# barry-mir/mixing-style-transfer

Hardware: AMD Instinct MI355X
Metric: triplets/sec (10 s @ 44.1 kHz, 4-stem, bs=24) (higher is better)
Workload: dtype f32

## Files before the change

include/mst.h:

```cpp
#ifndef MST_H_
#define MST_H_

#include <stddef.h>
#include <stdint.h>

#ifdef __cplusplus
extern "C" {
#endif

#define MST_ABI_VERSION 1

#define MST_OK 0
#define MST_EINVAL (-1)
#define MST_ENOMEM (-2)
#define MST_EHIP (-3)

int mst_version(void);
const char* mst_last_error(void);

typedef struct mst_plan mst_plan;

int mst_plan_create(mst_plan** out, int sample_rate, int n_fft, int hop, int n_mels,
                    const float* window, const float* fb, int detailed_bins);
void mst_plan_destroy(mst_plan* plan);
int mst_plan_frames(const mst_plan* plan, int T);
int mst_plan_feature_dim(const mst_plan* plan);
size_t mst_melfeat_workspace_bytes(const mst_plan* plan, int B, int T);

int mst_melfeat_forward(const mst_plan* plan, const float* stems, int B, int T, float* logmel,
                        float* feats, void* workspace, size_t workspace_bytes, void* stream);
int mst_melfeat_forward_stems(const mst_plan* plan, const float* const stems4[4], long long clip_stride,
                              int B, int T, float* logmel, float* feats, void* workspace,
                              size_t workspace_bytes, void* stream);
int mst_melfeat_forward_pcm16(const mst_plan* plan, const int16_t* stems, int B, int T, float* logmel,
                              float* feats, void* workspace, size_t workspace_bytes, void* stream);
int mst_melfeat_forward_stems_pcm16(const mst_plan* plan, const int16_t* const stems4[4], long long clip_stride,
                                    int B, int T, float* logmel, float* feats, void* workspace,
                                    size_t workspace_bytes, void* stream);

#define MST_LOGMEL_REF 0
#define MST_LOGMEL_CM32 1
#define MST_LOGMEL_CM16 2
int mst_plan_layout_supported(const mst_plan* plan, int layout);
typedef struct mst_melfeat_io {
  const void* stems4[4];
  long long clip_stride;
  int32_t pcm16;
  int32_t layout;
  void* logmel;
  void* logmel_lo;
  uint32_t* absmax;
  float* feats;
} mst_melfeat_io;
int mst_melfeat_forward_io(const mst_plan* plan, const mst_melfeat_io* io, int B, int T, void* workspace,
                           size_t workspace_bytes, void* stream);

typedef struct mst_encoder mst_encoder;

typedef struct mst_encoder_config {
  int32_t n_mels, split_size, overlap, n_subbands;
  int32_t feature_dim, embed_dim;
  int32_t film_hidden;
  int32_t attn_hidden;
  float bn_eps;
} mst_encoder_config;

// ... 177 lines not shown
```

mixing-style-transfer_amd/_lib.py:

```python
import ctypes as C
import os
import subprocess
import threading

_HERE = os.path.dirname(os.path.abspath(__file__))
LIB_PATH = os.environ.get("MST_LIB", os.path.join(_HERE, "libmst.so"))
CSRC = os.path.join(_HERE, "csrc")

MST_OK = 0


class MstError(RuntimeError):
    pass


class EncoderConfig(C.Structure):
    _fields_ = [("n_mels", C.c_int32), ("split_size", C.c_int32), ("overlap", C.c_int32),
                ("n_subbands", C.c_int32), ("feature_dim", C.c_int32), ("embed_dim", C.c_int32),
                ("film_hidden", C.c_int32), ("attn_hidden", C.c_int32), ("bn_eps", C.c_float)]


_W_FIELDS = ["conv1_w", "conv1_b", "bn1_w", "bn1_b", "bn1_mean", "bn1_var",
             "conv2_w", "conv2_b", "bn2_w", "bn2_b", "bn2_mean", "bn2_var",
             "mlp0_w", "mlp0_b", "mlp3_w", "mlp3_b", "head_w", "head_b",
# ... 51 lines not shown

class FilmPtrs(C.Structure):
    _fields_ = [(k, C.c_void_p) for k in ("mlp0_w", "mlp0_b", "mlp3_w", "mlp3_b", "head_w", "head_b")]


SYMBOLS = {
    "mst_version": (C.c_int, []),
    "mst_last_error": (C.c_char_p, []),
    "mst_plan_create": (C.c_int, [C.POINTER(C.c_void_p), C.c_int, C.c_int, C.c_int, C.c_int, C.c_void_p, C.c_void_p,
                                  C.c_int]),
    "mst_plan_destroy": (None, [C.c_void_p]),
    "mst_plan_frames": (C.c_int, [C.c_void_p, C.c_int]),
    "mst_plan_feature_dim": (C.c_int, [C.c_void_p]),
    "mst_melfeat_workspace_bytes": (C.c_size_t, [C.c_void_p, C.c_int, C.c_int]),
    "mst_melfeat_forward": (C.c_int, [C.c_void_p, C.c_void_p, C.c_int, C.c_int, C.c_void_p, C.c_void_p, C.c_void_p,
                                      C.c_size_t, C.c_void_p]),
    "mst_melfeat_forward_stems": (C.c_int, [C.c_void_p, C.POINTER(C.c_void_p), C.c_longlong, C.c_int, C.c_int,
                                            C.c_void_p, C.c_void_p, C.c_void_p, C.c_size_t, C.c_void_p]),
    "mst_melfeat_forward_pcm16": (C.c_int, [C.c_void_p, C.c_void_p, C.c_int, C.c_int, C.c_void_p, C.c_void_p,
                                            C.c_void_p, C.c_size_t, C.c_void_p]),
    "mst_melfeat_forward_stems_pcm16": (C.c_int, [C.c_void_p, C.POINTER(C.c_void_p), C.c_longlong, C.c_int, C.c_int,
                                                  C.c_void_p, C.c_void_p, C.c_void_p, C.c_size_t, C.c_void_p]),
    "mst_plan_layout_supported": (C.c_int, [C.c_void_p, C.c_int]),
    "mst_melfeat_forward_io": (C.c_int, [C.c_void_p, C.POINTER(MelfeatIO), C.c_int, C.c_int, C.c_void_p, C.c_size_t,
                                         C.c_void_p]),
    "mst_encoder_layout_supported": (C.c_int, [C.c_void_p, C.c_int]),
    "mst_encoder_forward_in": (C.c_int, [C.c_void_p, C.POINTER(LogmelIn), C.c_int, C.c_void_p, C.c_int, C.c_void_p,
                                         C.POINTER(EncoderTaps), C.c_void_p, C.c_size_t, C.c_void_p]),
    "mst_encoder_create": (C.c_int, [C.POINTER(C.c_void_p), C.POINTER(EncoderConfig), C.POINTER(EncoderWeights)]),
    "mst_encoder_destroy": (None, [C.c_void_p]),
    "mst_encoder_set_precision": (C.c_int, [C.c_void_p, C.c_int]),
    "mst_encoder_set_train_precision": (C.c_int, [C.c_void_p, C.c_int]),
    "mst_encoder_workspace_bytes": (C.c_size_t, [C.c_void_p, C.c_int, C.c_int]),
    "mst_encoder_forward": (C.c_int, [C.c_void_p, C.c_void_p, C.c_int, C.c_void_p, C.c_int, C.c_void_p,
                                      C.POINTER(EncoderTaps), C.c_void_p, C.c_size_t, C.c_void_p]),
    "mst_encoder_train_workspace_bytes": (C.c_size_t, [C.c_void_p, C.c_int, C.c_int]),
    "mst_encoder_forward_train": (C.c_int, [C.c_void_p, C.c_void_p, C.c_int, C.c_void_p, C.c_int, C.c_void_p,
                                            C.POINTER(EncoderTrainTaps), C.c_void_p, C.c_size_t, C.c_void_p]),
    "mst_dropout_mask": (C.c_int, [C.c_float, C.c_uint64, C.c_longlong, C.c_void_p, C.c_void_p]),
    "mst_head_save_bytes": (C.c_size_t, [C.POINTER(HeadDims), C.c_int, C.c_float]),
    "mst_head_backward_workspace_bytes": (C.c_size_t, [C.POINTER(HeadDims), C.c_int]),
    "mst_head_forward_train": (C.c_int, [C.POINTER(HeadDims), C.POINTER(HeadPtrs), C.c_void_p, C.c_int, C.c_float, C.c_uint64, C.c_float,
                                         C.c_uint64, C.c_void_p, C.c_void_p, C.c_size_t, C.c_void_p]),
    "mst_head_backward": (C.c_int, [C.POINTER(HeadDims), C.POINTER(HeadPtrs), C.c_void_p, C.c_int, C.c_float, C.c_uint64, C.c_float,
                                    C.c_uint64, C.c_void_p, C.c_void_p, C.POINTER(HeadPtrs), C.c_void_p, C.c_void_p, C.c_size_t, C.c_void_p]),
    "mst_film_save_bytes": (C.c_size_t, [C.POINTER(FilmDims), C.c_int]),
# ... 88 lines not shown
```

mixing-style-transfer_amd/csrc/fft_pk.h:

```cpp
#pragma once
#include <hip/hip_runtime.h>

namespace mstpk {

typedef float v2f __attribute__((ext_vector_type(2)));
typedef float v4f __attribute__((ext_vector_type(4)));

__device__ __forceinline__ v2f mk(float x, float y) {
  v2f r;
  r.x = x, r.y = y;
  return r;
}
__device__ __forceinline__ v2f add_mi(v2f a, v2f b) {
  v2f d;
  asm("v_pk_add_f32 %0, %1, %2 op_sel:[0,1] op_sel_hi:[1,0] neg_hi:[0,1]" : "=v"(d) : "v"(a), "v"(b));
  return d;
}
__device__ __forceinline__ v2f sub_mi(v2f a, v2f b) {
  v2f d;
  asm("v_pk_add_f32 %0, %1, %2 op_sel:[0,1] op_sel_hi:[1,0] neg_lo:[0,1]" : "=v"(d) : "v"(a), "v"(b));
  return d;
}
__device__ __forceinline__ v2f cmul(v2f a, v2f w) {
  v2f t, d;
// ... 100 lines not shown
    v2f* dst = scr + 144 * (lane >> 4) + (lane & 15);
#pragma unroll
    for (int u = 0; u < 2; ++u)
#pragma unroll
      for (int t = 0; t < 8; ++t) dst[576 * u + 16 * t] = x[8 * u + t];
  }
  __builtin_amdgcn_wave_barrier();
  {
    const v2f* sa = scr + lane;
    const v2f* sb = scr + jb_of(lane);
#pragma unroll
    for (int t = 0; t < 8; ++t) x[t] = sa[144 * t], x[8 + t] = sb[144 * t];
    fill2();
#pragma unroll
    for (int t = 1; t < 8; ++t) {
      x[t] = cmul(x[t], tw3[(t - 1) * 64 + lane]);
      x[8 + t] = cmul(x[8 + t], tw3[(7 + t - 1) * 64 + lane]);
    }
    dft8(x);
    dft8(x + 8);
  }
}

inline void fill_twiddles_host(float2* tw2, float2* tw3) {
  const double pi = 3.14159265358979323846;
  for (int t = 1; t < 8; ++t)
    for (int lane = 0; lane < 64; ++lane) {
      const double a = -2.0 * pi * (double)((lane & 15) * t) / 128.0;
      tw2[(t - 1) * 64 + lane] = make_float2((float)cos(a), (float)sin(a));
      for (int u = 0; u < 2; ++u) {
        const int j = u ? (lane ? 128 - lane : 64) : lane;
        const double b = -2.0 * pi * (double)(j * t) / 1024.0;
        tw3[(u * 7 + t - 1) * 64 + lane] = make_float2((float)cos(b), (float)sin(b));
      }
    }
}

}
```

mixing-style-transfer_amd/csrc/melfeat.hip:

```cpp
#include "common.h"
#include "fft_wave.h"
#include "fft_pk.h"

#include <algorithm>
#include <cmath>
#include <vector>


namespace {

constexpr int kWaves = 8;
constexpr int kFPW = 2;
constexpr int kTF = kWaves * kFPW;
constexpr int kTileStride = kTF + 1;
constexpr int kThreads = kWaves * 64;
constexpr int nf_of(int n_fft) { return n_fft >= 2048 ? 1 : kFPW; }
constexpr int kNumScalars = 80;

enum : int {
  S_LOGSUM = 0,
  S_LINSUM = 4,
  S_MASK = 8,
  S_SQ = 12,
  S_PEAK = 20,
// ... 919 lines not shown
    hipError_t e = hipFuncSetAttribute(reinterpret_cast<const void*>(melfeat_kernel<NFFT, NB, ST>),
                                       hipFuncAttributeMaxDynamicSharedMemorySize, (int)lds);
    if (e != hipSuccess) return e;
  }
  hipLaunchKernelGGL((melfeat_kernel<NFFT, NB, ST>), dim3(grid), dim3(kThreads), lds, st, kp);
  return hipGetLastError();
}

template <int NFFT, typename ST, int WPS>
hipError_t launch_melfeat_spw(const KParams& kp, int grid, size_t lds, hipStream_t st) {
  {
    hipError_t e = hipFuncSetAttribute(reinterpret_cast<const void*>(melfeat_spw_kernel<NFFT, ST, WPS>),
                                       hipFuncAttributeMaxDynamicSharedMemorySize, (int)lds);
    if (e != hipSuccess) return e;
  }
  hipLaunchKernelGGL((melfeat_spw_kernel<NFFT, ST, WPS>), dim3(grid), dim3(SpwGeom<WPS>::THREADS), lds, st, kp);
  return hipGetLastError();
}

template <int NFFT>
constexpr int tw_count_of() { return FftPlan<NFFT / 2>::TW; }

#include "melfeat_v2.inc"
#include "melfeat_v2_2048.inc"

}

struct mst_plan {
  int sr, n_fft, hop, n_mels, detailed_bins, feat_dim;
  int nc, nb, nnz, tw_count;
  int glen[4], goff[4];
  int batches_per_run;
  float* d_window = nullptr;
  float2* d_tw = nullptr;
  float2* d_tw2 = nullptr;
  int tw2_count = 0;
  float2* d_post = nullptr;
  float* d_melw = nullptr;
  LaneBand* d_lanebands = nullptr;
  bool v2_ok = false;
  int v2_nslot = 0, v2_glen[kV2Slots] = {0}, v2_goff[kV2Slots] = {0}, v2_segw_count = 0, v2_wps = 3, v2_maxcnt = 1;
  int2* d_v2_bandtab = nullptr;
  bool v4_ok = false;
  int v4_nslot = 0, v4_glen[4] = {0, 0, 0, 0}, v4_goff[4] = {0, 0, 0, 0}, v4_segw_count = 0, v4_maxcnt = 0;
  float2* d_v4_tw4 = nullptr;
  float2* d_v4_segw = nullptr;
  int* d_v4_pstart = nullptr;
  int* d_v4_pid = nullptr;
  int* d_v4_bandtab = nullptr;
  float2* d_v2_tw2 = nullptr;
  float2* d_v2_tw3 = nullptr;
  float2* d_v2_segw = nullptr;
  int* d_v2_segstart = nullptr;
  int* d_v2_segid = nullptr;
};

namespace {

void add_pass_tw(std::vector<float2>& tw, int NC, int R, int NS) {
  if (NS == 1) return;
  const int nbf = NS <= 64 ? 1 : NC / R / 64;
  for (int u = 0; u < nbf; ++u)
    for (int t = 1; t < R; ++t)
      for (int lane = 0; lane < 64; ++lane) {
// ... 9 lines not shown
    case 512: return {{8, 1}, {8, 8}, {8, 64}};
    case 1024: return {{8, 1}, {8, 8}, {4, 64}, {4, 256}};
  }
  return {};
}

int frames_per_run_of(const mst_plan* p, int , int F) {
  if (p->batches_per_run > 0) return p->batches_per_run * kTF;
  int fpr = (F + 31) / 32;
  fpr += fpr & 1;
  return std::max(2 * kTF, fpr);
}
int runs_per_clip(const mst_plan* p, int B, int F) {
  const int fpr = frames_per_run_of(p, B, F);
  return (F + fpr - 1) / fpr;
}
int pstride_of(const mst_plan* p) { return 4 * p->n_mels + kNumScalars; }

int v2_fpw(const mst_plan* p, int F) { return std::max(1, ((F + 31) / 32 + p->v2_wps - 1) / p->v2_wps); }
int v2_runs(const mst_plan* p, int F) {
  const int fpr = p->v2_wps * v2_fpw(p, F);
  return (F + fpr - 1) / fpr;
}

bool segment_bins(const float* fb, int n_bins, int M, std::vector<int>& seg, std::vector<float>& wl, std::vector<float>& wh) {
  std::vector<int> peak(M, -1);
  for (int m = 0; m < M; ++m) {
    float best = 0.f;
    for (int k = 0; k < n_bins; ++k)
      if (fb[(size_t)k * M + m] > best) best = fb[(size_t)k * M + m], peak[m] = k;
  }
  seg.assign(n_bins, 0), wl.assign(n_bins, 0.f), wh.assign(n_bins, 0.f);
  int prev = 0;
  for (int k = 0; k < n_bins; ++k) {
    int b0 = -1, b1 = -1, cnt = 0;
    for (int m = 0; m < M; ++m)
      if (fb[(size_t)k * M + m] != 0.0f) {
        if (cnt == 0) b0 = m;
        b1 = m;
        ++cnt;
      }
    if (cnt > 2 || (cnt == 2 && b1 != b0 + 1)) return false;
    int s = prev;
    if (cnt == 2) {
      s = b1, wl[k] = fb[(size_t)k * M + b0], wh[k] = fb[(size_t)k * M + b1];
    } else if (cnt == 1) {
// ... 177 lines not shown
  if (melw.empty()) melw.push_back(0.f);
  std::vector<float2> tw;
  for (auto pr : passes_of(p->nc)) add_pass_tw(tw, p->nc, pr.first, pr.second);
  p->tw_count = (int)tw.size();
  std::vector<float2> tw2;
  if (n_fft <= 1024)
    for (auto pr : passes_of(n_fft)) add_pass_tw(tw2, n_fft, pr.first, pr.second);
  p->tw2_count = (int)tw2.size();
  if (tw2.empty()) tw2.push_back(make_float2(1.f, 0.f));
  std::vector<float2> post(p->nc);
  for (int q = 0; q < p->nc / 64; ++q)
    for (int lane = 0; lane < 64; ++lane) {
      const int k = lane + 64 * q;
      const double a = -2.0 * M_PI * (double)k / (double)n_fft;
      post[(size_t)q * 64 + lane] = make_float2((float)cos(a), (float)sin(a));
    }
  {
    std::vector<float2> segw, t2(mstpk::kTw2Rows * 64), t3(mstpk::kTw3Rows * 64);
    std::vector<int> segstart, segid;
    std::vector<int2> bandtab;
    const char* w = getenv("MST_V2_WPS");
    p->v2_wps = ((w && atoi(w) == 2) || n_mels > 128) ? 2 : 3;
    p->v2_ok = n_fft == 1024 && hop == 256 && v2_build_segments(p, fb, segw, segstart, segid, bandtab);
    if (p->v2_ok) {
      mstpk::fill_twiddles_host(t2.data(), t3.data());
      int rc2;
      if ((rc2 = mst::upload(&p->d_v2_tw2, t2.data(), t2.size())) || (rc2 = mst::upload(&p->d_v2_tw3, t3.data(), t3.size())) ||
          (rc2 = mst::upload(&p->d_v2_segw, segw.data(), segw.size())) ||
          (rc2 = mst::upload(&p->d_v2_segstart, segstart.data(), segstart.size())) ||
          (rc2 = mst::upload(&p->d_v2_segid, segid.data(), segid.size())) ||
          (rc2 = mst::upload(&p->d_v2_bandtab, bandtab.data(), bandtab.size()))) {
        mst_plan_destroy(p);
        return rc2;
      }
    }
  }
  {
    std::vector<float2> segw, t2(mstpk::kTw2Rows * 64), t3(mstpk::kTw3Rows * 64), t4(16 * 64);
    std::vector<int> pstart, pid, bandtab;
    p->v4_ok = n_fft == 2048 && hop == 512 && v4_build_pieces(p, fb, segw, pstart, pid, bandtab);
    if (p->v4_ok) {
      mstpk::fill_twiddles_host(t2.data(), t3.data());
      for (int t = 0; t < 8; ++t)
        for (int lane = 0; lane < 64; ++lane)
          for (int u = 0; u < 2; ++u) {
            const int k = (u ? (lane ? 128 - lane : 64) : lane) + 128 * t;
// ... 22 lines not shown
  }
  *out = p;
  return MST_OK;
}

void mst_plan_destroy(mst_plan* p) {
  if (!p) return;
  (void)hipFree(p->d_window), (void)hipFree(p->d_tw), (void)hipFree(p->d_tw2), (void)hipFree(p->d_post), (void)hipFree(p->d_melw),
      (void)hipFree(p->d_lanebands);
  (void)hipFree(p->d_v2_tw2), (void)hipFree(p->d_v2_tw3), (void)hipFree(p->d_v2_segw), (void)hipFree(p->d_v2_segstart),
      (void)hipFree(p->d_v2_segid), (void)hipFree(p->d_v2_bandtab);
  (void)hipFree(p->d_v4_tw4), (void)hipFree(p->d_v4_segw), (void)hipFree(p->d_v4_pstart), (void)hipFree(p->d_v4_pid),
      (void)hipFree(p->d_v4_bandtab);
  delete p;
}

int mst_plan_frames(const mst_plan* p, int T) { return p ? 1 + T / p->hop : MST_EINVAL; }
int mst_plan_feature_dim(const mst_plan* p) { return p ? p->feat_dim : MST_EINVAL; }

size_t mst_melfeat_workspace_bytes(const mst_plan* p, int B, int T) {
  if (!p || B <= 0 || T <= 0) return 0;
  const int F = 1 + T / p->hop;
  const int runs = std::max(runs_per_clip(p, B, F), p->v2_ok ? v2_runs(p, F) : (p->v4_ok ? v4_runs(F) : 0));
  return mst::align_up((size_t)B * runs * pstride_of(p) * sizeof(float), 256);
}

}

namespace {
struct LogmelOut {
  int layout = MST_LOGMEL_REF;
  void* lo = nullptr;
  unsigned* absmax = nullptr;
};
int melfeat_forward_impl(const mst_plan* p, const void* const stems4[4], bool pcm16, long long clip_stride, int B, int T,
                         float* logmel, float* feats, void* workspace, size_t workspace_bytes, void* stream,
                         const LogmelOut& lo = LogmelOut());
bool plan_uses_v2(const mst_plan* p);
}

extern "C" {

int mst_melfeat_forward(const mst_plan* p, const float* stems, int B, int T, float* logmel, float* feats,
                        void* workspace, size_t workspace_bytes, void* stream) {
  MST_REQUIRE(p && stems, "mst_melfeat_forward: NULL plan/stems");
  const void* four[4] = {stems, stems + 2 * (size_t)T, stems + 4 * (size_t)T, stems + 6 * (size_t)T};
  return melfeat_forward_impl(p, four, false, (long long)8 * T, B, T, logmel, feats, workspace, workspace_bytes, stream);
// ... 118 lines not shown
                        (size_t)v4::kWPS * v4::kBLK * 4 * 128 * sizeof(float) + 16;
    MST_REQUIRE(lds4 <= 160 * 1024, "mst_melfeat_forward: LDS %zu B exceeds 160 KiB", lds4);
    const int grid4 = B * k4.runs_per_clip;
    e = pcm16 ? launch_melfeat_v2_2048<short>(k4, grid4, lds4, st) : launch_melfeat_v2_2048<float>(k4, grid4, lds4, st);
  } else if (use_v2) {
    K2Params k2{};
    for (int i = 0; i < 4; ++i) k2.stem[i] = stems4[i];
    k2.clip_stride = clip_stride, k2.logmel = logmel, k2.partials = reinterpret_cast<float*>(workspace);
    k2.out_mode = lmo.layout, k2.logmel_lo = lmo.lo, k2.absmax = lmo.absmax;
    k2.window = p->d_window, k2.tw2 = p->d_v2_tw2, k2.tw3 = p->d_v2_tw3, k2.segw = p->d_v2_segw;
    k2.segstart = p->d_v2_segstart, k2.segid = p->d_v2_segid, k2.bandtab = p->d_v2_bandtab, k2.maxcnt = p->v2_maxcnt;
    k2.B = B, k2.T = T, k2.F = F, k2.M = p->n_mels;
    k2.nslot = p->v2_nslot, k2.segw_count = p->v2_segw_count;
    for (int r = 0; r < kV2Slots; ++r) k2.glen[r] = p->v2_glen[r], k2.goff[r] = p->v2_goff[r];
    k2.fpw = v2_fpw(p, F), k2.runs_per_clip = v2_runs(p, F), k2.pstride = pstride_of(p);
    kp.runs_per_clip = k2.runs_per_clip;
    const int wps = p->v2_wps;
    const bool wide = p->n_mels > 128;
    const size_t lds2 = (size_t)((mstpk::kTw2Rows + mstpk::kTw3Rows) * 64 + p->v2_segw_count + 4 * wps * mstpk::kScr) * sizeof(float2) +
                        (size_t)(wps * (wide ? 4 : (wps == 2 ? 8 : 4)) * 4 * (wide ? 256 : 128) + 1024) * sizeof(float) + 16;
    MST_REQUIRE(lds2 <= 160 * 1024, "mst_melfeat_forward: LDS %zu B exceeds 160 KiB", lds2);
    const int grid2 = B * k2.runs_per_clip;
    if (wide) e = pcm16 ? launch_melfeat_v2<short, 2, 4>(k2, grid2, lds2, st) : launch_melfeat_v2<float, 2, 4>(k2, grid2, lds2, st);
    else if (wps == 3) {
      const bool stdt = v2_table_is_standard(p) && !getenv("MST_V2_NOSTD");
      e = pcm16 ? launch_melfeat_v2<short, 3>(k2, grid2, lds2, st, stdt) : launch_melfeat_v2<float, 3>(k2, grid2, lds2, st, stdt);
    }
    else e = pcm16 ? launch_melfeat_v2<short, 2>(k2, grid2, lds2, st) : launch_melfeat_v2<float, 2>(k2, grid2, lds2, st);
  } else {
  const int grid = B * kp.runs_per_clip;
  const int wps = getenv("MST_SPW_WPS") ? atoi(getenv("MST_SPW_WPS")) : 3;
  auto spw_lds = [&](int w) {
    return (size_t)(nc + p->tw2_count + 4 * w * (p->n_fft + p->n_fft / 8)) * sizeof(float2) +
           (size_t)(((p->nnz + 3) & ~3) + (w == 2 ? 16 : 6) * (8 * p->n_mels + 1)) * sizeof(float);
  };
  const bool spw_ok = kp.vec_ok && kp.vec4_ok && p->hop * 4 == p->n_fft && p->n_mels <= 128 && p->nb == 2 &&
                      (p->n_fft == 512 || p->n_fft == 1024) && !getenv("MST_MELFEAT_GENERIC");
  const bool spw3 = spw_ok && wps == 3 && p->n_fft == 1024 && spw_lds(3) <= 160 * 1024;
  const bool spw = spw3 || (spw_ok && spw_lds(2) <= 160 * 1024);
  if (spw3) {
    e = pcm16 ? launch_melfeat_spw<1024, short, 3>(kp, grid, spw_lds(3), st) : launch_melfeat_spw<1024, float, 3>(kp, grid, spw_lds(3), st);
  } else if (spw) {
    const size_t lds_spw = spw_lds(2);
    if (p->n_fft == 1024)
      e = pcm16 ? launch_melfeat_spw<1024, short, 2>(kp, grid, lds_spw, st) : launch_melfeat_spw<1024, float, 2>(kp, grid, lds_spw, st);
    else
      e = pcm16 ? launch_melfeat_spw<512, short, 2>(kp, grid, lds_spw, st) : launch_melfeat_spw<512, float, 2>(kp, grid, lds_spw, st);
  } else {
#define MST_CASE(NF)                                                                                          \
// ... 26 lines not shown
```

mixing-style-transfer_amd/csrc/melfeat_v2.inc:

```

constexpr int kV2Slots = 6;

struct K2Params {
  const void* stem[4];
  long long clip_stride;
  float* logmel;
  void* logmel_lo;
  unsigned* absmax;
  int out_mode;
  float* partials;
  const float* window;
  const float2* tw2;
  const float2* tw3;
  const float2* segw;
  const int* segstart;
  const int* segid;
  const int2* bandtab;
  int B, T, F, M;
  int nslot, glen[kV2Slots], goff[kV2Slots], segw_count;
  int maxcnt;
  int fpw;
  int runs_per_clip, pstride;
};

namespace v2 {
using namespace mstpk;

constexpr int kP2 = 0;
constexpr int kExN = 288;
constexpr int kExDump = kExN - 1;
constexpr int kExHi = 544;
constexpr int kExLo = kExHi + kExN;
static_assert(kExLo + kExN <= kScr, "exchange areas must fit the FFT scratch");
// ... 401 lines not shown
```

mixing-style-transfer_amd/mixing_utils.py:

```python
import ctypes as C

import numpy as np
import torch

from . import _lib

STEMS = ("vocals", "bass", "drums", "other")

FEATURES_DEFERRED = -32768.0


def deferred_features(feature_dim: int) -> torch.Tensor:
    return torch.full((feature_dim,), FEATURES_DEFERRED, dtype=torch.float32)


def is_deferred(features: torch.Tensor) -> torch.Tensor:
    return features[..., :1] == FEATURES_DEFERRED


def detailed_bins_for_feature_dim(feature_dim: int):
    if feature_dim < 8 or (feature_dim - 8) % 4:
        return None
    sd = (feature_dim - 8) // 4 - 9
    if sd == 5:
# ... 15 lines not shown
    slope = hz.unsqueeze(0) - freqs.unsqueeze(1)
    lower = (-1.0 * slope[:, :-2]) / dhz[:-1]
    upper = slope[:, 2:] / dhz[1:]
    return torch.max(torch.zeros(1), torch.min(lower, upper))


class LogMel:

    def __init__(self, layout, data, lo=None, absmax=None):
        self.layout, self.data, self.lo, self.absmax = layout, data, lo, absmax
        self.B, self.frames, self.n_mels = data.shape[0], data.shape[1], data.shape[2]
        self.device = data.device

    def to_reference(self):
        if self.layout == _lib.LOGMEL_CM16 and self.lo is None:
            raise _lib.MstError("this LogMel holds the float16 HIGH parts only (what the plain-float16 kernels read): the fp32 "
                                "log-mel cannot be recovered from it -- ask stage A for the reference layout instead")
        x = self.data.float() if self.lo is None else self.data.float() + self.lo.float()
        return x.permute(0, 3, 2, 1).contiguous()


class MelFeatPlan:

    def __init__(self, sample_rate, n_fft, hop_length, n_mels, detailed_bins=0, window=None, fb=None):
        self.sample_rate, self.n_fft, self.hop_length, self.n_mels = sample_rate, n_fft, hop_length, n_mels
        self.window = (hann_window(n_fft) if window is None else window).detach().float().cpu().contiguous()
        self.fb = (melscale_fbanks_htk(n_fft // 2 + 1, n_mels, sample_rate) if fb is None else fb)
        self.fb = self.fb.detach().float().cpu().contiguous()
        h = C.c_void_p()
        L = _lib.lib()
        _lib.check(L.mst_plan_create(C.byref(h), sample_rate, n_fft, hop_length, n_mels,
                                     C.c_void_p(self.window.data_ptr()), C.c_void_p(self.fb.data_ptr()),
                                     int(detailed_bins)), "mst_plan_create")
        self._h = h
        self.feature_dim = L.mst_plan_feature_dim(h)
        self._ws = None

    def __del__(self):
        h, self._h = getattr(self, "_h", None), None
        if h:
            try:
                _lib.lib().mst_plan_destroy(h)
            except Exception:
                pass

    def frames(self, T: int) -> int:
        return 1 + T // self.hop_length

    def _workspace(self, B, T, device):
        need = _lib.lib().mst_melfeat_workspace_bytes(self._h, B, T)
        if self._ws is None or self._ws.numel() < need or self._ws.device != device:
            self._ws = torch.empty(need, dtype=torch.uint8, device=device)
        return self._ws, need

    def supports_layout(self, layout) -> bool:
        return bool(_lib.lib().mst_plan_layout_supported(self._h, int(layout)))

# ... 327 lines not shown
```

Before: 2772.

## Add paired-frame stage-A kernel splitting each run into sub-runs with a combine pass

```diff
diff --git a/include/mst.h b/include/mst.h
--- a/include/mst.h
+++ b/include/mst.h
@@ -42,6 +42,10 @@
 #define MST_LOGMEL_CM32 1
 #define MST_LOGMEL_CM16 2
 int mst_plan_layout_supported(const mst_plan* plan, int layout);
+
+#define MST_STAGE_A_PAIRS 0
+#define MST_STAGE_A_SINGLE 1
+int mst_plan_set_stage_a(mst_plan* plan, int kernel);
 typedef struct mst_melfeat_io {
   const void* stems4[4];
   long long clip_stride;
diff --git a/mixing-style-transfer_amd/_lib.py b/mixing-style-transfer_amd/_lib.py
--- a/mixing-style-transfer_amd/_lib.py
+++ b/mixing-style-transfer_amd/_lib.py
@@ -97,6 +97,7 @@
     "mst_melfeat_forward_stems_pcm16": (C.c_int, [C.c_void_p, C.POINTER(C.c_void_p), C.c_longlong, C.c_int, C.c_int,
                                                   C.c_void_p, C.c_void_p, C.c_void_p, C.c_size_t, C.c_void_p]),
     "mst_plan_layout_supported": (C.c_int, [C.c_void_p, C.c_int]),
+    "mst_plan_set_stage_a": (C.c_int, [C.c_void_p, C.c_int]),
     "mst_melfeat_forward_io": (C.c_int, [C.c_void_p, C.POINTER(MelfeatIO), C.c_int, C.c_int, C.c_void_p, C.c_size_t,
                                          C.c_void_p]),
     "mst_encoder_layout_supported": (C.c_int, [C.c_void_p, C.c_int]),
diff --git a/mixing-style-transfer_amd/csrc/fft_pk.h b/mixing-style-transfer_amd/csrc/fft_pk.h
--- a/mixing-style-transfer_amd/csrc/fft_pk.h
+++ b/mixing-style-transfer_amd/csrc/fft_pk.h
@@ -146,6 +146,87 @@
   }
 }
 
+template <class F1 = NoFill, class F2 = NoFill>
+__device__ __forceinline__ void fft1024x2(v2f (&xa)[16], v2f (&xb)[16], v2f* scr, const v2f* tw2, const v2f* tw3, int lane,
+                                          F1 fill1 = F1(), F2 fill2 = F2()) {
+  v4f* const row = reinterpret_cast<v4f*>(scr + 18 * lane);
+  const int m = lane & 15;
+  const v2f* const src1 = scr + 18 * (lane >> 4) + (m >> 2) + 4 * (m & 3);
+  v2f* const dst2 = scr + 144 * (lane >> 4) + (lane & 15);
+  const v2f* const sa = scr + lane;
+  const v2f* const sb = scr + jb_of(lane);
+  auto put1 = [&](const v2f (&x)[16]) __attribute__((always_inline)) {
+#pragma unroll
+    for (int q = 0; q < 8; ++q) {
+      v4f w;
+      w.x = x[2 * q].x, w.y = x[2 * q].y, w.z = x[2 * q + 1].x, w.w = x[2 * q + 1].y;
+      row[q] = w;
+    }
+  };
+  auto get1 = [&](v2f (&x)[16]) __attribute__((always_inline)) {
+#pragma unroll
+    for (int u = 0; u < 2; ++u)
+#pragma unroll
+      for (int t = 0; t < 8; ++t) x[8 * u + t] = src1[72 * u + 144 * t];
+  };
+  auto put2 = [&](const v2f (&x)[16]) __attribute__((always_inline)) {
+#pragma unroll
+    for (int u = 0; u < 2; ++u)
+#pragma unroll
+      for (int t = 0; t < 8; ++t) dst2[576 * u + 16 * t] = x[8 * u + t];
+  };
+  auto get2 = [&](v2f (&x)[16]) __attribute__((always_inline)) {
+#pragma unroll
+    for (int t = 0; t < 8; ++t) x[t] = sa[144 * t], x[8 + t] = sb[144 * t];
+  };
+  v2f w2[8], w3[16];
+  auto pass2 = [&](v2f (&x)[16]) __attribute__((always_inline)) {
+#pragma unroll
+    for (int t = 1; t < 8; ++t) {
+      x[t] = cmul(x[t], w2[t]);
+      x[8 + t] = cmul(x[8 + t], w2[t]);
+    }
+    dft8(x);
+    dft8(x + 8);
+  };
+  auto pass3 = [&](v2f (&x)[16]) __attribute__((always_inline)) {
+#pragma unroll
+    for (int t = 1; t < 8; ++t) {
+      x[t] = cmul(x[t], w3[t]);
+      x[8 + t] = cmul(x[8 + t], w3[8 + t]);
+    }
+    dft8(x);
+    dft8(x + 8);
+  };
+  dft16(xa);
+  put1(xa);
+  __builtin_amdgcn_wave_barrier();
+  get1(xa);
+#pragma unroll
+  for (int t = 1; t < 8; ++t) w2[t] = tw2[(t - 1) * 64 + lane];
+  dft16(xb);
+  __builtin_amdgcn_wave_barrier();
+  put1(xb);
+  __builtin_amdgcn_wave_barrier();
+  get1(xb);
+  fill1();
+  pass2(xa);
+  __builtin_amdgcn_wave_barrier();
+  put2(xa);
+  __builtin_amdgcn_wave_barrier();
+  get2(xa);
+#pragma unroll
+  for (int t = 1; t < 8; ++t) w3[t] = tw3[(t - 1) * 64 + lane], w3[8 + t] = tw3[(7 + t - 1) * 64 + lane];
+  pass2(xb);
+  __builtin_amdgcn_wave_barrier();
+  put2(xb);
+  __builtin_amdgcn_wave_barrier();
+  get2(xb);
+  fill2();
+  pass3(xa);
+  pass3(xb);
+}
+
 inline void fill_twiddles_host(float2* tw2, float2* tw3) {
   const double pi = 3.14159265358979323846;
   for (int t = 1; t < 8; ++t)
diff --git a/mixing-style-transfer_amd/csrc/melfeat.hip b/mixing-style-transfer_amd/csrc/melfeat.hip
--- a/mixing-style-transfer_amd/csrc/melfeat.hip
+++ b/mixing-style-transfer_amd/csrc/melfeat.hip
@@ -965,6 +965,7 @@
 constexpr int tw_count_of() { return FftPlan<NFFT / 2>::TW; }
 
 #include "melfeat_v2.inc"
+#include "melfeat_v2_pair.inc"
 #include "melfeat_v2_2048.inc"
 
 }
@@ -983,6 +984,8 @@
   LaneBand* d_lanebands = nullptr;
   bool v2_ok = false;
   int v2_nslot = 0, v2_glen[kV2Slots] = {0}, v2_goff[kV2Slots] = {0}, v2_segw_count = 0, v2_wps = 3, v2_maxcnt = 1;
+  bool v2_std = false;
+  int stage_a = MST_STAGE_A_PAIRS;
   int2* d_v2_bandtab = nullptr;
   bool v4_ok = false;
   int v4_nslot = 0, v4_glen[4] = {0, 0, 0, 0}, v4_goff[4] = {0, 0, 0, 0}, v4_segw_count = 0, v4_maxcnt = 0;
@@ -1038,6 +1041,7 @@
   const int fpr = p->v2_wps * v2_fpw(p, F);
   return (F + fpr - 1) / fpr;
 }
+bool v2_pairs(const mst_plan* p) { return p->v2_ok && p->v2_std && p->v2_wps == 3 && p->stage_a == MST_STAGE_A_PAIRS; }
 
 bool segment_bins(const float* fb, int n_bins, int M, std::vector<int>& seg, std::vector<float>& wl, std::vector<float>& wh) {
   std::vector<int> peak(M, -1);
@@ -1261,6 +1265,7 @@
     const char* w = getenv("MST_V2_WPS");
     p->v2_wps = ((w && atoi(w) == 2) || n_mels > 128) ? 2 : 3;
     p->v2_ok = n_fft == 1024 && hop == 256 && v2_build_segments(p, fb, segw, segstart, segid, bandtab);
+    p->v2_std = p->v2_ok && v2_table_is_standard(p) && !getenv("MST_V2_NOSTD");
     if (p->v2_ok) {
       mstpk::fill_twiddles_host(t2.data(), t3.data());
       int rc2;
@@ -1329,7 +1334,15 @@
   if (!p || B <= 0 || T <= 0) return 0;
   const int F = 1 + T / p->hop;
   const int runs = std::max(runs_per_clip(p, B, F), p->v2_ok ? v2_runs(p, F) : (p->v4_ok ? v4_runs(F) : 0));
-  return mst::align_up((size_t)B * runs * pstride_of(p) * sizeof(float), 256);
+  const size_t sub = v2_pairs(p) ? (size_t)B * v2_runs(p, F) * v2p::kSubRuns * 4 * v2p::kSubStride * sizeof(float) : 0;
+  return mst::align_up((size_t)B * runs * pstride_of(p) * sizeof(float), 256) + mst::align_up(sub, 256);
+}
+
+int mst_plan_set_stage_a(mst_plan* p, int kernel) {
+  MST_REQUIRE(p, "mst_plan_set_stage_a: NULL plan");
+  MST_REQUIRE(kernel == MST_STAGE_A_PAIRS || kernel == MST_STAGE_A_SINGLE, "mst_plan_set_stage_a: unknown kernel %d", kernel);
+  p->stage_a = kernel;
+  return MST_OK;
 }
 
 }
@@ -1494,9 +1507,14 @@
     MST_REQUIRE(lds2 <= 160 * 1024, "mst_melfeat_forward: LDS %zu B exceeds 160 KiB", lds2);
     const int grid2 = B * k2.runs_per_clip;
     if (wide) e = pcm16 ? launch_melfeat_v2<short, 2, 4>(k2, grid2, lds2, st) : launch_melfeat_v2<float, 2, 4>(k2, grid2, lds2, st);
-    else if (wps == 3) {
-      const bool stdt = v2_table_is_standard(p) && !getenv("MST_V2_NOSTD");
-      e = pcm16 ? launch_melfeat_v2<short, 3>(k2, grid2, lds2, st, stdt) : launch_melfeat_v2<float, 3>(k2, grid2, lds2, st, stdt);
+    else if (v2_pairs(p)) {
+      k2.sub = reinterpret_cast<float*>(static_cast<char*>(workspace) +
+                                        mst::align_up((size_t)B * k2.runs_per_clip * k2.pstride * sizeof(float), 256));
+      MST_REQUIRE(v2p_lds_bytes(k2.segw_count) <= 80 * 1024, "mst_melfeat_forward: LDS %zu B exceeds 80 KiB (two workgroups per CU)",
+                  v2p_lds_bytes(k2.segw_count));
+      e = pcm16 ? launch_melfeat_v2p<short>(k2, feats != nullptr, st) : launch_melfeat_v2p<float>(k2, feats != nullptr, st);
+    } else if (wps == 3) {
+      e = pcm16 ? launch_melfeat_v2<short, 3>(k2, grid2, lds2, st, p->v2_std) : launch_melfeat_v2<float, 3>(k2, grid2, lds2, st, p->v2_std);
     }
     else e = pcm16 ? launch_melfeat_v2<short, 2>(k2, grid2, lds2, st) : launch_melfeat_v2<float, 2>(k2, grid2, lds2, st);
   } else {
diff --git a/mixing-style-transfer_amd/csrc/melfeat_v2.inc b/mixing-style-transfer_amd/csrc/melfeat_v2.inc
--- a/mixing-style-transfer_amd/csrc/melfeat_v2.inc
+++ b/mixing-style-transfer_amd/csrc/melfeat_v2.inc
@@ -9,6 +9,7 @@
   unsigned* absmax;
   int out_mode;
   float* partials;
+  float* sub;
   const float* window;
   const float2* tw2;
   const float2* tw3;
diff --git a/mixing-style-transfer_amd/csrc/melfeat_v2_pair.inc b/mixing-style-transfer_amd/csrc/melfeat_v2_pair.inc
--- /dev/null
+++ b/mixing-style-transfer_amd/csrc/melfeat_v2_pair.inc
@@ -0,0 +1,418 @@
+
+namespace v2p {
+constexpr int kSubRuns = 3;
+constexpr int kSubStride = 2 * 64 + 16;
+constexpr int kBLK = 4;
+}
+
+template <typename ST, bool CM>
+__global__ __launch_bounds__(256) __attribute__((amdgpu_waves_per_eu(2, 2))) void melfeat_v2p_kernel(const K2Params p) {
+#pragma clang fp contract(off)
+  using namespace mstpk;
+  using namespace v2;
+  using namespace v2p;
+  constexpr int NBL = 2, BLK = kBLK, SB = kBLK, MB = 128, M = 128;
+  constexpr float kLn2 = 0.69314718055994530942f;
+  extern __shared__ __attribute__((aligned(16))) unsigned char smem[];
+  v2f* s_tw2 = reinterpret_cast<v2f*>(smem);
+  v2f* s_tw3 = s_tw2 + kTw2Rows * 64;
+  v2f* s_segw = s_tw3 + kTw3Rows * 64;
+  float* s_win = reinterpret_cast<float*>(s_segw + p.segw_count);
+  float* exch = s_win + 1024;
+  v2f* s_scr = reinterpret_cast<v2f*>(exch + BLK * 4 * MB);
+  unsigned* s_amax = reinterpret_cast<unsigned*>(s_scr + 4 * kScr);
+  const int T = p.T;
+  constexpr int kStdLen0 = 14, kStdLen1 = 3, kStdOff1 = 14;
+
+  const int tid = threadIdx.x, lane = tid & 63;
+  const int stem = __builtin_amdgcn_readfirstlane(tid >> 6);
+  const int work = mst::xcd_remap(blockIdx.x, gridDim.x);
+  const int crun = work / kSubRuns, h = work % kSubRuns;
+  const int clip = crun / p.runs_per_clip, run = crun % p.runs_per_clip;
+  const int f_begin = run * kSubRuns * p.fpw;
+  const int f_end = min(p.F, f_begin + kSubRuns * p.fpw);
+  {
+    const v2f* g2 = reinterpret_cast<const v2f*>(p.tw2);
+    const v2f* g3 = reinterpret_cast<const v2f*>(p.tw3);
+    const v2f* gs = reinterpret_cast<const v2f*>(p.segw);
+    for (int i = tid; i < kTw2Rows * 64; i += 256) s_tw2[i] = g2[i];
+    for (int i = tid; i < kTw3Rows * 64; i += 256) s_tw3[i] = g3[i];
+    for (int i = tid; i < p.segw_count; i += 256) s_segw[i] = gs[i];
+    for (int i = tid; i < 1024; i += 256) s_win[i] = p.window[i];
+    if (tid == 0) *s_amax = 0u;
+  }
+  auto chan = [&](int c) {
+    return static_cast<const ST*>(p.stem[c >> 1]) + (size_t)clip * p.clip_stride + (size_t)(c & 1) * T;
+  };
+  const ST* const xL = chan(2 * stem);
+  const ST* const xR = chan(2 * stem + 1);
+  const int o_piv = min(f_begin * 256, T - 1);
+  const float pvL = Smp<ST>::ld(xL + o_piv), pvR = Smp<ST>::ld(xR + o_piv);
+  v2f* scr = s_scr + stem * kScr;
+  int seg_start[3], seg_id[3];
+#pragma unroll
+  for (int r = 0; r < 3; ++r) seg_start[r] = p.segstart[r * 64 + lane], seg_id[r] = p.segid[r * 64 + lane];
+  const int jb = jb_of(lane);
+  const bool l0 = lane == 0;
+
+  float acc_db[NBL], acc_log = 0.f, acc_lin = 0.f, acc_mask = 0.f, mixsq = 0.f;
+#pragma unroll
+  for (int r = 0; r < NBL; ++r) acc_db[r] = 0.f;
+  float sqL = 0.f, sqR = 0.f, pkL = 0.f, pkR = 0.f, dsL = 0.f, dsR = 0.f, dqL = 0.f, dqR = 0.f;
+  float cr = 0.f, mid = 0.f, side = 0.f;
+
+  const int f0 = f_begin + h * p.fpw;
+  const int nfw = max(0, min(p.fpw, f_end - f0));
+  auto ld2 = [&](int pos) {
+    const int q = reflect_idx(pos, T);
+    return mk(ld_at(xL, q), ld_at(xR, q));
+  };
+  v2f raw[20];
+#pragma unroll
+  for (int t = 0; t < 20; ++t) raw[t] = mk(0.f, 0.f);
+  {
+    const int b0 = f0 * 256 - 512 + lane;
+    if (nfw > 0)
+#pragma unroll
+      for (int t = 0; t < 16; ++t) raw[t] = ld2(b0 + 64 * t);
+    if (nfw > 1)
+#pragma unroll
+      for (int t = 16; t < 20; ++t) raw[t] = ld2(b0 + 64 * t);
+  }
+  __syncthreads();
+
+  constexpr int kMixLead = 2;
+#pragma unroll
+  for (int k = 0; k < kMixLead; ++k) {
+    const int mp0 = (f0 + k) * 256 + 64 * stem + lane;
+    if (k < nfw && mp0 < T) {
+      float c8[8];
+#pragma unroll
+      for (int c = 0; c < 8; ++c) c8[c] = ld_at(chan(c), mp0);
+      const float mL = ((c8[0] + c8[2]) + c8[4]) + c8[6];
+      const float mR = ((c8[1] + c8[3]) + c8[5]) + c8[7];
+      mixsq = fmaf(mL, mL, mixsq);
+      mixsq = fmaf(mR, mR, mixsq);
+    }
+  }
+
+  const int nblk = (p.fpw + BLK - 1) / BLK;
+  float out[2 * NBL][SB];
+#pragma unroll
+  for (int k = 0; k < 2 * NBL; ++k)
+#pragma unroll
+    for (int e = 0; e < SB; ++e) out[k][e] = 0.f;
+  auto store_block = [&](int fb0, int cnt) __attribute__((always_inline)) {
+    if (!p.logmel || CM) return;
+#pragma unroll
+    for (int r = 0; r < NBL; ++r) {
+      const int b = lane + 64 * r;
+#pragma unroll
+      for (int c = 0; c < 2; ++c) {
+        float* dst = p.logmel + (((size_t)clip * 8 + 2 * stem + c) * M + b) * p.F + fb0;
+        const float* o = out[2 * r + c];
+        if (cnt == 4) {
+          *reinterpret_cast<f4u*>(dst) = f4u{o[0], o[1], o[2], o[3]};
+        } else {
+#pragma unroll
+          for (int q = 0; q < 3; ++q)
+            if (q < cnt) dst[q] = o[q];
+        }
+      }
+    }
+  };
+  auto put_p2 = [&](const v2f (&xx)[16], float ia, float ib) __attribute__((always_inline)) {
+    const v2f sc4 = mk(0.25f * ia, 0.25f * ib);
+    v2f* P2 = scr + kP2;
+#pragma unroll
+    for (int t = 0; t < 4; ++t) {
+      const v2f zm_a = sel2(1ull, xx[(8 - t) & 7], xx[15 - t]);
+      const v2f zm_b = sel2(1ull, xx[15 - t], xx[7 - t]);
+      P2[lane + 128 * t] = pair_power4(xx[t], zm_a) * sc4;
+      P2[jb + 128 * t] = pair_power4(xx[8 + t], zm_b) * sc4;
+    }
+    if (l0) P2[512] = xx[4] * xx[4] * mk(ia, ib);
+    if (lane < 16) P2[513 + lane] = mk(0.f, 0.f);
+  };
+  auto walk = [&](const v2f (&wv)[kStdLen0 + kStdLen1]) __attribute__((always_inline)) {
+    const v2f* pp0 = scr + kP2 + seg_start[0];
+    const v2f* pp1 = scr + kP2 + seg_start[1];
+    v2f q0[kStdLen0], q1[kStdLen1];
+#pragma unroll
+    for (int k = 0; k < kStdLen0; ++k) q0[k] = pp0[k];
+#pragma unroll
+    for (int k = 0; k < kStdLen1; ++k) q1[k] = pp1[k];
+    v2f slo = mk(0.f, 0.f), shi = mk(0.f, 0.f);
+#pragma unroll
+    for (int k = 0; k < kStdLen0; ++k) slo = bcast_fma(wv[k].x, q0[k], slo), shi = bcast_fma(wv[k].y, q0[k], shi);
+    scr[kExHi + seg_id[0]] = shi;
+    scr[kExLo + seg_id[0]] = slo;
+    slo = mk(0.f, 0.f), shi = mk(0.f, 0.f);
+#pragma unroll
+    for (int k = 0; k < kStdLen1; ++k)
+      slo = bcast_fma(wv[kStdOff1 + k].x, q1[k], slo), shi = bcast_fma(wv[kStdOff1 + k].y, q1[k], shi);
+    scr[kExHi + seg_id[1]] = shi;
+    scr[kExLo + seg_id[1]] = slo;
+    scr[kExHi + seg_id[2]] = mk(0.f, 0.f);
+    scr[kExLo + seg_id[2]] = mk(0.f, 0.f);
+  };
+  auto get_bands = [&](v2f (&m)[NBL]) __attribute__((always_inline)) {
+#pragma unroll
+    for (int r = 0; r < NBL; ++r) {
+      const int b = lane + 64 * r;
+      m[r] = scr[kExHi + min(b, kExDump)] + scr[kExLo + min(b + 1, kExDump)];
+    }
+  };
+
+  int blk = 0;
+  auto step = [&](auto ic, bool hasB) __attribute__((always_inline)) {
+    constexpr int I = decltype(ic)::value;
+    const int f = f0 + blk * BLK + I;
+    const int fi = blk * BLK + I;
+    v2f x[2][16];
+    float ia[2], ib[2];
+    {
+      float wv[16];
+#pragma unroll
+      for (int t = 0; t < 16; ++t) wv[t] = s_win[lane + 64 * t];
+#pragma unroll
+      for (int n = 0; n < 2; ++n) {
+        float ma = 0.f, mb = 0.f;
+#pragma unroll
+        for (int t = 0; t < 16; ++t) {
+          x[n][t] = raw[t + 4 * n] * mk(wv[t], wv[t]);
+          ma = fmaxf(ma, fabsf(x[n][t].x)), mb = fmaxf(mb, fabsf(x[n][t].y));
+        }
+        const unsigned ua = wave_umax_uniform(__float_as_uint(ma)), ub = wave_umax_uniform(__float_as_uint(mb));
+        int sh = 0;
+        if (ua != 0u && ub != 0u) sh = max(-40, min(40, (int)(ua >> 23) - (int)(ub >> 23)));
+        if (sh != 0) {
+          const float sc = __uint_as_float((unsigned)(127 + sh) << 23);
+#pragma unroll
+          for (int t = 0; t < 16; ++t) x[n][t].y *= sc;
+        }
+        ia[n] = ua != 0u ? 1.0f : 0.f;
+        ib[n] = ub != 0u ? __uint_as_float((unsigned)(127 - 2 * sh) << 23) : 0.f;
+      }
+    }
+    v2f nxt[8];
+    {
+      const bool n1 = fi + 2 < nfw, n2 = fi + 3 < nfw;
+      const int base2 = f * 256 + 768, b2 = base2 + lane;
+      if (n2 && base2 + 511 < T) {
+#pragma unroll
+        for (int j = 0; j < 8; ++j) nxt[j] = mk(ld_at(xL, b2 + 64 * j), ld_at(xR, b2 + 64 * j));
+      } else {
+#pragma unroll
+        for (int j = 0; j < 8; ++j) nxt[j] = ((j < 4) ? n1 : n2) ? ld2(b2 + 64 * j) : mk(0.f, 0.f);
+      }
+    }
+    float mx[2][8];
+    int mp[2];
+#pragma unroll
+    for (int n = 0; n < 2; ++n) {
+      mp[n] = fi + n + kMixLead < nfw ? (f + n + kMixLead) * 256 + 64 * stem + lane : T;
+      const int q = min(mp[n], T - 1);
+#pragma unroll
+      for (int c = 0; c < 8; ++c) mx[n][c] = ld_at(chan(c), q);
+    }
+    auto moments = [&](int n) __attribute__((always_inline)) {
+#pragma unroll
+      for (int j = 0; j < 4; ++j) {
+        const bool mk_ = (f + n) * 256 + lane + 64 * j < T;
+        const v2f s = raw[8 + j + 4 * n];
+        const float L = mk_ ? s.x : 0.f, Rr = mk_ ? s.y : 0.f;
+        const float dL = mk_ ? L - pvL : 0.f, dR = mk_ ? Rr - pvR : 0.f;
+        sqL = fmaf(L, L, sqL), sqR = fmaf(Rr, Rr, sqR);
+        pkL = fmaxf(pkL, fabsf(L)), pkR = fmaxf(pkR, fabsf(Rr));
+        dsL += dL, dsR += dR;
+        dqL = fmaf(dL, dL, dqL), dqR = fmaf(dR, dR, dqR);
+        cr = fmaf(dL, dR, cr);
+        mid = fmaf(L + Rr, L + Rr, mid);
+        side = fmaf(L - Rr, L - Rr, side);
+      }
+    };
+    auto mixture = [&](int n) __attribute__((always_inline)) {
+      if (mp[n] < T) {
+        const float mL = ((mx[n][0] + mx[n][2]) + mx[n][4]) + mx[n][6];
+        const float mR = ((mx[n][1] + mx[n][3]) + mx[n][5]) + mx[n][7];
+        mixsq = fmaf(mL, mL, mixsq);
+        mixsq = fmaf(mR, mR, mixsq);
+      }
+    };
+    auto fill1 = [&]() __attribute__((always_inline)) {
+      moments(0);
+      if (hasB) moments(1);
+    };
+    auto fill2 = [&]() __attribute__((always_inline)) {
+      mixture(0);
+      mixture(1);
+    };
+    __builtin_amdgcn_wave_barrier();
+    fft1024x2(x[0], x[1], scr, s_tw2, s_tw3, lane, fill1, fill2);
+    auto bands = [&](const v2f (&m)[NBL], int n) __attribute__((always_inline)) {
+#pragma unroll
+      for (int r = 0; r < NBL; ++r) {
+        const int b = lane + 64 * r;
+        const float l0v = __log2f(m[r].x + 1e-10f) * kLn2, l1v = __log2f(m[r].y + 1e-10f) * kLn2;
+        out[2 * r][(I + n) % SB] = l0v, out[2 * r + 1][(I + n) % SB] = l1v;
+        acc_db[r] += l0v + l1v;
+        acc_log += l0v + l1v;
+        acc_lin += m[r].x + m[r].y;
+        exch[((I + n) * 4 + stem) * MB + b] = 0.5f * (m[r].x + m[r].y);
+      }
+    };
+    __builtin_amdgcn_wave_barrier();
+    put_p2(x[0], ia[0], ib[0]);
+    __builtin_amdgcn_wave_barrier();
+    v2f wv[kStdLen0 + kStdLen1];
+#pragma unroll
+    for (int k = 0; k < kStdLen0 + kStdLen1; ++k) wv[k] = s_segw[k * 64 + lane];
+    walk(wv);
+    __builtin_amdgcn_wave_barrier();
+    put_p2(x[1], ia[1], ib[1]);
+    v2f mA[NBL];
+    get_bands(mA);
+    __builtin_amdgcn_wave_barrier();
+    walk(wv);
+    bands(mA, 0);
+    __builtin_amdgcn_wave_barrier();
+    if (hasB) {
+      v2f mB[NBL];
+      get_bands(mB);
+      bands(mB, 1);
+    }
+    __builtin_amdgcn_wave_barrier();
+#pragma unroll
+    for (int t = 0; t < 12; ++t) raw[t] = raw[t + 8];
+#pragma unroll
+    for (int j = 0; j < 8; ++j) raw[12 + j] = nxt[j];
+  };
+#pragma unroll 1
+  for (blk = 0; blk < nblk; ++blk) {
+    const int nv = max(0, min(BLK, nfw - blk * BLK));
+    if (nv > 0) step(std::integral_constant<int, 0>(), nv > 1);
+    if (nv > 2) step(std::integral_constant<int, 2>(), nv > 3);
+    {
+      const int done = min(nfw, (blk + 1) * BLK);
+      if (nv > 0 && (done % SB == 0 || done == nfw)) {
+        const int cnt = (done - 1) % SB + 1;
+        store_block(f0 + done - cnt, cnt);
+      }
+    }
+    __syncthreads();
+#pragma unroll
+    for (int r = 0; r < NBL; ++r) {
+      const int b = lane + 64 * r;
+#pragma unroll 2
+      for (int e = 0; e < nv; ++e) {
+        float other = -INFINITY, own = 0.f;
+#pragma unroll
+        for (int j = 0; j < 4; ++j) {
+          const float sj = exch[(e * 4 + j) * MB + b];
+          other = (j != stem) ? fmaxf(other, sj) : other;
+          own = (j == stem) ? sj : own;
+        }
+        acc_mask += __builtin_amdgcn_rcpf(1.0f + __expf(own - other));
+      }
+    }
+    if (CM && p.absmax) block_absmax<NBL, BLK>(out, lane, nv, M, s_amax);
+    if (CM && p.logmel) cm_stage<NBL, BLK, 1, kScr>(out, s_scr, 0, stem, lane, nv, p.out_mode);
+    __syncthreads();
+    if (CM && p.logmel)
+      cm_store<NBL, BLK>(scr, stem, lane, nv, ((size_t)clip * p.F + (f0 + blk * BLK)) * M, M, p.logmel, p.logmel_lo, p.out_mode);
+  }
+
+  float* rec = p.sub + (((size_t)clip * p.runs_per_clip + run) * kSubRuns + h) * 4 * kSubStride + stem * kSubStride;
+#pragma unroll
+  for (int r = 0; r < NBL; ++r) rec[r * 64 + lane] = acc_db[r];
+  {
+    const float v[13] = {acc_log, acc_lin, sqL, sqR, dsL, dsR, dqL, dqR, cr, mid, side, mixsq, acc_mask};
+#pragma unroll
+    for (int k = 0; k < 13; ++k) {
+      const float r = mst::wave_sum(v[k]);
+      if (lane == 0) rec[128 + k] = r;
+    }
+    const float a = mst::wave_max(pkL), b = mst::wave_max(pkR);
+    if (lane == 0) rec[128 + 13] = a, rec[128 + 14] = b;
+  }
+  if (CM && p.absmax) {
+    __syncthreads();
+    if (tid == 0) atomicMax(p.absmax + clip, *s_amax);
+  }
+}
+
+template <typename ST>
+__global__ __launch_bounds__(256) void melfeat_v2p_combine_kernel(const K2Params p) {
+  using namespace v2p;
+  constexpr int M = 128;
+  const int clip = blockIdx.x / p.runs_per_clip, run = blockIdx.x % p.runs_per_clip, tid = threadIdx.x, T = p.T;
+  const float* sub = p.sub + (size_t)blockIdx.x * kSubRuns * 4 * kSubStride;
+  float* part = p.partials + (size_t)blockIdx.x * p.pstride;
+  const int f_begin = run * kSubRuns * p.fpw, f_end = min(p.F, f_begin + kSubRuns * p.fpw);
+  for (int i = tid; i < 4 * M; i += 256) {
+    const int s = i / M, b = i % M;
+    float v = 0.f;
+#pragma unroll
+    for (int w = 0; w < kSubRuns; ++w) v += sub[(w * 4 + s) * kSubStride + b];
+    part[s * M + b] = v;
+  }
+  if (tid < 4) {
+    const int s = tid;
+    float v[13], pk0 = 0.f, pk1 = 0.f;
+#pragma unroll
+    for (int k = 0; k < 13; ++k) v[k] = 0.f;
+    for (int w = 0; w < kSubRuns; ++w) {
+      const float* a = sub + (w * 4 + s) * kSubStride + 128;
+#pragma unroll
+      for (int k = 0; k < 13; ++k) v[k] += a[k];
+      pk0 = fmaxf(pk0, a[13]), pk1 = fmaxf(pk1, a[14]);
+    }
+    float* q = part + 4 * M;
+    q[S_LOGSUM + s] = v[0];
+    q[S_LINSUM + s] = v[1];
+    q[S_SQ + 2 * s] = v[2], q[S_SQ + 2 * s + 1] = v[3];
+    q[S_DSUM + 2 * s] = v[4], q[S_DSUM + 2 * s + 1] = v[5];
+    q[S_DSQ + 2 * s] = v[6], q[S_DSQ + 2 * s + 1] = v[7];
+    q[S_CROSS + s] = v[8];
+    q[S_MID + s] = v[9];
+    q[S_SIDE + s] = v[10];
+    q[S_MASK + s] = v[12];
+    q[S_PEAK + 2 * s] = pk0, q[S_PEAK + 2 * s + 1] = pk1;
+    const int o_piv = min(f_begin * 256, T - 1);
+    const ST* x = static_cast<const ST*>(p.stem[s]) + (size_t)clip * p.clip_stride;
+    q[S_PIVOT + 2 * s] = Smp<ST>::ld(x + o_piv), q[S_PIVOT + 2 * s + 1] = Smp<ST>::ld(x + T + o_piv);
+  }
+  if (tid == 8) {
+    float mxs = 0.f;
+    for (int s = 0; s < 4; ++s)
+      for (int w = 0; w < kSubRuns; ++w) mxs += sub[(w * 4 + s) * kSubStride + 128 + 11];
+    const int o_begin = f_begin * 256, o_end = (f_end == p.F) ? T : min(T, f_end * 256);
+    part[4 * M + S_MIX] = mxs;
+    part[4 * M + S_NSAMP] = (float)max(0, o_end - o_begin);
+    part[4 * M + S_NFRAME] = (float)max(0, f_end - f_begin);
+  }
+}
+
+inline size_t v2p_lds_bytes(int segw_count) {
+  return (size_t)((mstpk::kTw2Rows + mstpk::kTw3Rows) * 64 + segw_count + 4 * mstpk::kScr) * sizeof(float2) +
+         (size_t)(1024 + v2p::kBLK * 4 * 128) * sizeof(float) + 16;
+}
+template <typename ST>
+hipError_t launch_melfeat_v2p(const K2Params& kp, bool combine, hipStream_t st) {
+  const size_t lds = v2p_lds_bytes(kp.segw_count);
+  const int grid = kp.B * kp.runs_per_clip * v2p::kSubRuns;
+  hipError_t e;
+  if (kp.out_mode != 0) {
+    e = hipFuncSetAttribute(reinterpret_cast<const void*>(melfeat_v2p_kernel<ST, true>), hipFuncAttributeMaxDynamicSharedMemorySize, (int)lds);
+    if (e != hipSuccess) return e;
+    hipLaunchKernelGGL((melfeat_v2p_kernel<ST, true>), dim3(grid), dim3(256), lds, st, kp);
+  } else {
+    e = hipFuncSetAttribute(reinterpret_cast<const void*>(melfeat_v2p_kernel<ST, false>), hipFuncAttributeMaxDynamicSharedMemorySize, (int)lds);
+    if (e != hipSuccess) return e;
+    hipLaunchKernelGGL((melfeat_v2p_kernel<ST, false>), dim3(grid), dim3(256), lds, st, kp);
+  }
+  if ((e = hipGetLastError()) != hipSuccess || !combine) return e;
+  hipLaunchKernelGGL((melfeat_v2p_combine_kernel<ST>), dim3(kp.B * kp.runs_per_clip), dim3(256), 0, st, kp);
+  return hipGetLastError();
+}
diff --git a/mixing-style-transfer_amd/mixing_utils.py b/mixing-style-transfer_amd/mixing_utils.py
--- a/mixing-style-transfer_amd/mixing_utils.py
+++ b/mixing-style-transfer_amd/mixing_utils.py
@@ -61,7 +61,9 @@
 
 class MelFeatPlan:
 
-    def __init__(self, sample_rate, n_fft, hop_length, n_mels, detailed_bins=0, window=None, fb=None):
+    STAGE_A = {"pairs": 0, "single": 1}
+
+    def __init__(self, sample_rate, n_fft, hop_length, n_mels, detailed_bins=0, window=None, fb=None, stage_a="pairs"):
         self.sample_rate, self.n_fft, self.hop_length, self.n_mels = sample_rate, n_fft, hop_length, n_mels
         self.window = (hann_window(n_fft) if window is None else window).detach().float().cpu().contiguous()
         self.fb = (melscale_fbanks_htk(n_fft // 2 + 1, n_mels, sample_rate) if fb is None else fb)
@@ -72,6 +74,7 @@
                                      C.c_void_p(self.window.data_ptr()), C.c_void_p(self.fb.data_ptr()),
                                      int(detailed_bins)), "mst_plan_create")
         self._h = h
+        _lib.check(L.mst_plan_set_stage_a(h, self.STAGE_A[stage_a]), "mst_plan_set_stage_a")
         self.feature_dim = L.mst_plan_feature_dim(h)
         self._ws = None
 
```

Result: no change. 2785 (median of 6 runs) (+0.5%).
